# visionworkbench/visionworkbench

Hardware: AMD Instinct MI355X
Metric: disparity Mpix/s, 4096x4096 pair, 7x7 SAD, +-64-px search (higher is better)
Workload: dtype u8

## Files before the change

visionworkbench_amd/csrc/bm_sad_u8.hip:

```cpp
#include <climits>
#include <cstdlib>
#include <type_traits>

#include "vwgpu_internal.h"
#include "u8_tile.h"

#ifdef VWGPU_TILE_STAMPS
__device__ unsigned long long* g_sad_stamps = nullptr;
extern "C" int vwgpu_debug_set_sad_stamps(void* d_buf) {
  unsigned long long* p = static_cast<unsigned long long*>(d_buf);
  return hipMemcpyToSymbol(HIP_SYMBOL(g_sad_stamps), &p, sizeof p) == hipSuccess ? 0 : -3;
}
#define VWGPU_STAMP(k) do { if (g_sad_stamps && tid == 0) g_sad_stamps[(size_t)wg * 16 + (k)] = wall_clock64(); } while (0)
#else
#define VWGPU_STAMP(k) do { } while (0)
#endif

namespace {

using namespace vwgpu_u8;
typedef uint32_t u32;
typedef uint64_t u64;
typedef unsigned short u16x2 __attribute__((ext_vector_type(2)));

__device__ __forceinline__ u32 pk_sub_u16(u32 a, u32 b) {
  return __builtin_bit_cast(u32, (u16x2)(__builtin_bit_cast(u16x2, a) - __builtin_bit_cast(u16x2, b)));
}
__device__ __forceinline__ u32 pk_max_u16(u32 a, u32 b) {
  return __builtin_bit_cast(u32, __builtin_elementwise_max(__builtin_bit_cast(u16x2, a), __builtin_bit_cast(u16x2, b)));
}
__device__ __forceinline__ u32 pk_min_u16(u32 a, u32 b) {
  return __builtin_bit_cast(u32, __builtin_elementwise_min(__builtin_bit_cast(u16x2, a), __builtin_bit_cast(u16x2, b)));
}
__device__ __forceinline__ void umin3_acc(u32& k, u32 a, u32 b) {
  asm volatile("v_min3_u32 %0, %0, %1, %2" : "+v"(k) : "v"(a), "v"(b));
}

template <int W>
__device__ __forceinline__ void key_sub(u32& key, u32 a, u32 b) {
  if (W == 0)
    asm volatile("v_sub_u16_sdwa %0, %1, %2 dst_sel:WORD_1 dst_unused:UNUSED_PRESERVE src0_sel:WORD_0 src1_sel:WORD_0"
                 : "+v"(key) : "v"(a), "v"(b));
  else
    asm volatile("v_sub_u16_sdwa %0, %1, %2 dst_sel:WORD_1 dst_unused:UNUSED_PRESERVE src0_sel:WORD_1 src1_sel:WORD_1"
                 : "+v"(key) : "v"(a), "v"(b));
}

template <int KX, int KY, int TY, int WV = 0>
struct Cfg {
  static constexpr int NW = (KX + 3) / 4;
  static constexpr int EW = NW <= 2 ? 2 : 4;
  static constexpr int WAVES = WV ? WV : (NW <= 2 ? 4 : 2);
  static constexpr int THREADS = WAVES * 64;
  static constexpr int TWB = WAVES * 256;
  static constexpr int NR = TY + KY - 1;
  static constexpr int LBW = TWB / 4 + NW + 1;
  static constexpr u32 LAST_MASK = (KX % 4 == 0) ? 0xffffffffu : ((1u << (8 * (KX % 4))) - 1u);
};

__device__ __forceinline__ void divmod_small(int idx, int d, float inv, int& quo, int& rem) {
  int qq = (int)(((float)idx + 0.5f) * inv);
  int rr = idx - qq * d;
  if (rr < 0) { --qq; rr += d; }
  if (rr >= d) { ++qq; rr -= d; }
  quo = qq; rem = rr;
}

__host__ __device__ constexpr size_t ent_words(int nr, int ne, int ew, int gr, int ty, int pt) {
  const size_t ent = (size_t)nr * ne * ew;
  const size_t merge = gr > 1 ? (size_t)(gr - 1) * (ty / gr) * 4 * pt + (size_t)gr * pt : 0;
  const size_t ob = (size_t)gr * (pt / 64) * 768;
  return ent > merge ? (ent > ob ? ent : ob) : (merge > ob ? merge : ob);
}

template <int KX, int KY, int TY, int GR, int WV = 0, bool EM = true>
__global__ void __launch_bounds__((GR * (Cfg<KX, KY, TY, WV>::THREADS)), (GR > 1 ? 1 : (TY <= 8 && KX <= 8 ? 3 : 2)))
bm_sad_u8_kernel(const float* __restrict__ L, ptrdiff_t ls, int lw, int lh,
                 const float* __restrict__ R, ptrdiff_t rs, int rcw, int rch,
                 int sx, int sy, int ne, int32_t* __restrict__ out, ptrdiff_t os, int ow, int oh,
                 int* __restrict__ flag_set, int* __restrict__ flag_clear,
                 int gxt, int ntiles, int last_round) {
  typedef Cfg<KX, KY, TY, WV> C;
  constexpr bool SPLIT = GR > 1;
  constexpr int NW = C::NW, EW = C::EW, NR = C::NR;
  constexpr int NRP = EM ? (NR | 1) : NR;
  extern __shared__ __attribute__((aligned(16))) u32 lds[];
  u32* ent = lds;
  const int bpitch = ne + NW + 1;
  u32* base = lds + ent_words(NRP, ne, EW, GR, TY, C::THREADS);
  u32* item_ctr = base + (size_t)NR * bpitch;

  constexpr int PT = C::THREADS;
  constexpr int NT = GR * PT;
  const int tid = threadIdx.x;
  const int grp = SPLIT ? __builtin_amdgcn_readfirstlane(tid / PT) : 0;
  const int ltid = SPLIT ? tid % PT : tid;
  const int pair_id = __builtin_amdgcn_readfirstlane(ltid >> 6);
  const int per_xcd = gridDim.x >> 3;
  const int wg = (int)(blockIdx.x & 7) * per_xcd + (int)(blockIdx.x >> 3);
  if (wg >= ntiles) return;
  const int x0 = (wg % gxt) * C::TWB;
  const int y0 = (wg / gxt) * TY;
  const int q = x0 + 4 * ltid;
  u32 bad_acc = 0;
  if (wg == 0 && tid == 0) *flag_clear = 0;
#ifdef VWGPU_TILE_STAMPS
  if (g_sad_stamps && tid == 0) {
    unsigned hw, xcc;
    asm volatile("s_getreg_b32 %0, hwreg(HW_REG_HW_ID)" : "=s"(hw));
    asm volatile("s_getreg_b32 %0, hwreg(HW_REG_XCC_ID)" : "=s"(xcc));
    unsigned long long* rec = g_sad_stamps + (size_t)wg * 16;
    rec[0] = wall_clock64(); rec[1] = clock64(); rec[2] = ((unsigned long long)xcc << 32) | hw;
  }
#endif

  stage_u8_rows<NR>(L, ls, lw, lh, x0, y0, C::LBW, C::LBW, ent, tid, NT, bad_acc);
  stage_u8_rows<NR>(R, rs, rcw, rch, x0, y0, bpitch, bpitch, base, tid, NT, bad_acc);
  __syncthreads();
  u64 win[NR][NW];
#pragma unroll
  for (int r = 0; r < NR; ++r) {
    u32 a[NW + 1];
#pragma unroll
    for (int n = 0; n <= NW; ++n) a[n] = ent[r * C::LBW + ltid + n];
#pragma unroll
    for (int n = 0; n < NW; ++n) win[r][n] = (u64)a[n] | ((u64)a[n + 1] << 32);
  }

  VWGPU_STAMP(3);
  u32 K[TY][4];
  u32 MN[TY][2], MX[TY][2];
#pragma unroll
  for (int y = 0; y < TY; ++y) K[y][0] = K[y][1] = K[y][2] = K[y][3] = 0xffffffffu;
  u32 eq_rows = (1u << TY) - 1u;
  int eq_checks = 0;
  constexpr int NPROBE = 4;
  const u32 zero = 0;

  const bool late = !SPLIT && (int)blockIdx.x >= last_round;
  if (!SPLIT) { if (late) __builtin_amdgcn_s_setprio(2); else __builtin_amdgcn_s_setprio(3); }
  typedef std::true_type T;
  typedef std::false_type F;

  auto sweep = [&](auto max_tag) __attribute__((always_inline)) {
    constexpr bool MAXSWEEP = decltype(max_tag)::value;
    for (int dy = 0; dy < sy; ++dy) {
      __syncthreads();
      if (dy > 0 || (MAXSWEEP && sy > 1)) stage_u8_rows<NR>(R, rs, rcw, rch, x0, y0 + dy, bpitch, bpitch, base, tid, NT, bad_acc);
      for (int t = 0; t < 4; ++t) {
        const int a_last = (sx + 2 - t) >> 2;
        __syncthreads();
        if (!MAXSWEEP && !SPLIT && dy == 0 && late) {
          if (t == 2) __builtin_amdgcn_s_setprio(1);
          else if (t == 3) __builtin_amdgcn_s_setprio(0);
        }
        {
          auto build = [&](int r, int m) __attribute__((always_inline)) {
            const u32* bp = base + (size_t)r * bpitch + m;
            u32 b[NW + 1];
#pragma unroll
            for (int n = 0; n <= NW; ++n) b[n] = bp[n];
            u32 w[EW];
#pragma unroll
            for (int n = 0; n < EW; ++n) w[n] = 0;
#pragma unroll
            for (int n = 0; n < NW; ++n) w[n] = __builtin_amdgcn_alignbyte(b[n + 1], b[n], t);
            w[NW - 1] &= C::LAST_MASK;
            u32* e = ent + (EM ? (size_t)m * NRP + r : (size_t)r * ne + m) * EW;
            if (EW == 2) *reinterpret_cast<uint2*>(e) = make_uint2(w[0], w[1]);
            else *reinterpret_cast<uint4*>(e) = make_uint4(w[0], w[1], w[2 % EW], w[3 % EW]);
          };
#pragma unroll 4
          for (int r = grp; r < NR; r += NT / PT) build(r, ltid);
          const int rem = ne - PT, total = NR * rem;
          const float inv = 1.0f / (float)rem;
          for (int idx = tid; idx < total; idx += NT) {
            int r, m;
            divmod_small(idx, rem, inv, r, m);
            build(r, PT + m);
          }
          if (SPLIT && tid < PT / 64) item_ctr[tid] = 0u;
        }
        __syncthreads();

        auto step = [&](int a, auto masked_tag, auto pair_tag, auto probe_tag) __attribute__((always_inline)) {
          constexpr bool MASKED = decltype(masked_tag)::value;
          constexpr bool PAIR = decltype(pair_tag)::value;
          constexpr bool PROBE = decltype(probe_tag)::value;
          const int jbase = 4 * a + t;
          const int ibase = dy * sx + jbase;
          u32 kinA[4], kinB[4];
          u32 orA[2] = {0u, 0u};
#pragma unroll
          for (int i = 0; i < 4; ++i) {
            kinA[i] = (u32)(ibase - i) & 0xffffu;
            kinB[i] = (u32)(ibase + 4 - i) & 0xffffu;
            if (MASKED) {
              const int d = jbase - i;
              if (d < 0 || d >= sx) orA[i >> 1] |= (i & 1) ? 0xffff0000u : 0x0000ffffu;
            }
          }
          const u32* ep = ent + (size_t)(ltid + a) * (EM ? NRP * EW : EW);
          u64 accA = 0, accB = 0;
          u64 PA[NR], PB[NR];
          constexpr int PF = 4;
          u32 wa[NR][EW], wb[NR][EW];
          auto fetch = [&](int r) __attribute__((always_inline)) {
            const u32* e = ep + (EM ? (size_t)r * EW : (size_t)r * ne * EW);
            constexpr int NX = EM ? NRP * EW : EW;
            if (EW == 2) {
              const uint2 v = *reinterpret_cast<const uint2*>(e);
              wa[r][0] = v.x; wa[r][1] = v.y;
              if (PAIR) { const uint2 u = *reinterpret_cast<const uint2*>(e + NX); wb[r][0] = u.x; wb[r][1] = u.y; }
            } else {
              const uint4 v = *reinterpret_cast<const uint4*>(e);
              wa[r][0] = v.x; wa[r][1] = v.y; wa[r][2 % EW] = v.z; wa[r][3 % EW] = v.w;
              if (PAIR) { const uint4 u = *reinterpret_cast<const uint4*>(e + NX); wb[r][0] = u.x; wb[r][1] = u.y; wb[r][2 % EW] = u.z; wb[r][3 % EW] = u.w; }
            }
          };
#pragma unroll
          for (int r = 0; r < PF && r < NR; ++r) fetch(r);
#pragma unroll
          for (int r = 0; r < NR; ++r) {
            if (r + PF < NR) fetch(r + PF);
#pragma unroll
            for (int n = 0; n < NW; ++n) {
              accA = __builtin_amdgcn_qsad_pk_u16_u8(win[r][n], wa[r][n], accA);
              if (PAIR) accB = __builtin_amdgcn_qsad_pk_u16_u8(win[r][n], wb[r][n], accB);
            }
            PA[r] = accA;
            if (PAIR) PB[r] = accB;
            if (r >= KY - 1) {
              const int y = r - (KY - 1);
              const int ro = (r >= KY) ? r - KY : 0;
              const u32 nA0 = (u32)PA[r], nA1 = (u32)(PA[r] >> 32);
              const u32 oA0 = (r >= KY) ? (u32)PA[ro] : zero;
              const u32 oA1 = (r >= KY) ? (u32)(PA[ro] >> 32) : zero;
              if (MAXSWEEP) {
                const u32 sA0 = pk_sub_u16(nA0, oA0), sA1 = pk_sub_u16(nA1, oA1);
                MN[y][0] = pk_min_u16(MN[y][0], MASKED ? (sA0 | orA[0]) : sA0);
                MN[y][1] = pk_min_u16(MN[y][1], MASKED ? (sA1 | orA[1]) : sA1);
                MX[y][0] = pk_max_u16(MX[y][0], MASKED ? (sA0 & ~orA[0]) : sA0);
                MX[y][1] = pk_max_u16(MX[y][1], MASKED ? (sA1 & ~orA[1]) : sA1);
                if (PAIR) {
                  const u32 nB0 = (u32)PB[r], nB1 = (u32)(PB[r] >> 32);
                  const u32 oB0 = (r >= KY) ? (u32)PB[ro] : zero;
                  const u32 oB1 = (r >= KY) ? (u32)(PB[ro] >> 32) : zero;
                  const u32 sB0 = pk_sub_u16(nB0, oB0), sB1 = pk_sub_u16(nB1, oB1);
                  MN[y][0] = pk_min_u16(MN[y][0], sB0);
                  MN[y][1] = pk_min_u16(MN[y][1], sB1);
                  MX[y][0] = pk_max_u16(MX[y][0], sB0);
                  MX[y][1] = pk_max_u16(MX[y][1], sB1);
                }
              } else {
                key_sub<0>(kinA[0], nA0, oA0); key_sub<1>(kinA[1], nA0, oA0);
                key_sub<0>(kinA[2], nA1, oA1); key_sub<1>(kinA[3], nA1, oA1);
                if (PAIR) {
                  const u32 nB0 = (u32)PB[r], nB1 = (u32)(PB[r] >> 32);
                  const u32 oB0 = (r >= KY) ? (u32)PB[ro] : zero;
                  const u32 oB1 = (r >= KY) ? (u32)(PB[ro] >> 32) : zero;
                  key_sub<0>(kinB[0], nB0, oB0); key_sub<1>(kinB[1], nB0, oB0);
                  key_sub<0>(kinB[2], nB1, oB1); key_sub<1>(kinB[3], nB1, oB1);
                  if (PROBE) {
                    u32 x[4];
#pragma unroll
                    for (int i = 0; i < 4; ++i) {
                      asm volatile("v_xor_b32 %0, %1, %2" : "=v"(x[i]) : "v"(kinA[i]), "v"(kinB[i]));
                      x[i] = (q + i < ow) ? x[i] : 0xffffffffu;
                    }
                    const u32 m01 = x[0] < x[1] ? x[0] : x[1], m23 = x[2] < x[3] ? x[2] : x[3];
                    if ((m01 < m23 ? m01 : m23) >> 16) eq_rows &= ~(1u << y);
                  }
                  umin3_acc(K[y][0], kinA[0], kinB[0]);
                  umin3_acc(K[y][1], kinA[1], kinB[1]);
                  umin3_acc(K[y][2], kinA[2], kinB[2]);
                  umin3_acc(K[y][3], kinA[3], kinB[3]);
                } else {
                  const u32 kA0 = (MASKED && (orA[0] & 0x0000ffffu)) ? 0xffffffffu : kinA[0];
                  const u32 kA1 = (MASKED && (orA[0] & 0xffff0000u)) ? 0xffffffffu : kinA[1];
                  const u32 kA2 = (MASKED && (orA[1] & 0x0000ffffu)) ? 0xffffffffu : kinA[2];
                  const u32 kA3 = (MASKED && (orA[1] & 0xffff0000u)) ? 0xffffffffu : kinA[3];
                  umin3_acc(K[y][0], kA0, kA0);
                  umin3_acc(K[y][1], kA1, kA1);
                  umin3_acc(K[y][2], kA2, kA2);
                  umin3_acc(K[y][3], kA3, kA3);
                }
              }
            }
          }
        };

        int a_lo = (t >= 3) ? 0 : 1;
        int a_hi = (sx - 1 - t >= 0) ? ((sx - 1 - t) >> 2) + 1 : 0;
        if (a_hi > a_last + 1) a_hi = a_last + 1;
        if (a_lo > a_hi) a_lo = a_hi;
        const int n1 = a_lo;
        const int npair = (a_hi - n1) > 0 ? (a_hi - n1) >> 1 : 0;
        int nprobe = 0;
        if (!MAXSWEEP && dy == 0 && t == 0) nprobe = npair < NPROBE - eq_checks ? npair : NPROBE - eq_checks;
        const int a4 = n1 + 2 * npair;
        const int n4 = a_last - a4 + 1 > 0 ? a_last - a4 + 1 : 0;
        const int nitems = n1 + npair + n4;
        int seq = 0;
        auto next_item = [&]() __attribute__((always_inline)) -> int {
          if (MAXSWEEP) return grp == 0 ? seq++ : 0x7fffffff;
          if (!SPLIT) return seq++;
          int lane, v = 0;
          asm volatile("v_mbcnt_lo_u32_b32 %0, -1, 0\n\tv_mbcnt_hi_u32_b32 %0, -1, %0" : "=v"(lane));
          if (lane == 0) v = (int)atomicAdd(&item_ctr[pair_id], 1u);
          return __builtin_amdgcn_readfirstlane(v);
        };
        int i = next_item();
        for (; i < n1; i = next_item()) step(i, T{}, F{}, F{});
        for (; i < n1 + nprobe; i = next_item()) step(n1 + 2 * (i - n1), F{}, T{}, T{});
        for (; i < n1 + npair; i = next_item()) step(n1 + 2 * (i - n1), F{}, T{}, F{});
        for (; i < nitems; i = next_item()) step(a4 + (i - n1 - npair), T{}, F{}, F{});
        eq_checks += nprobe;
        if (!MAXSWEEP && dy == 0) VWGPU_STAMP(4 + t);
      }
    }
  };
  sweep(F{});
  if (!SPLIT) __builtin_amdgcn_s_setprio(3);

  if (bad_acc != 0u) atomicOr(flag_set, 1);
  constexpr int RG = TY / GR;
  static_assert(TY % GR == 0, "rows per group");
  auto row_mine = [&](int y) __attribute__((always_inline)) -> bool { return !SPLIT || (y / RG == grp); };
  if (SPLIT) {
    u32* xk = ent;
    u32* xe = ent + (size_t)(GR - 1) * RG * 4 * PT;
    u32 eq_all = eq_rows;
#pragma unroll
    for (int d = 0; d < GR; ++d) {
      __syncthreads();
      if (grp != d) {
        const int slot = grp < d ? grp : grp - 1;
#pragma unroll
        for (int y = 0; y < RG; ++y)
#pragma unroll
          for (int s2 = 0; s2 < 4; ++s2) xk[((slot * RG + y) * 4 + s2) * PT + ltid] = K[d * RG + y][s2];
      }
      if (d == 0) xe[grp * PT + ltid] = eq_rows;
      __syncthreads();
      if (grp == d) {
#pragma unroll
        for (int slot = 0; slot < GR - 1; ++slot)
#pragma unroll
          for (int y = 0; y < RG; ++y)
#pragma unroll
            for (int s2 = 0; s2 < 4; ++s2) {
              const u32 o = xk[((slot * RG + y) * 4 + s2) * PT + ltid];
              K[d * RG + y][s2] = o < K[d * RG + y][s2] ? o : K[d * RG + y][s2];
            }
      }
      if (d == 0) {
#pragma unroll
        for (int g2 = 0; g2 < GR; ++g2) eq_all &= xe[g2 * PT + ltid];
      }
    }
    eq_rows = eq_all;
  }
  u32 cand = eq_checks < NPROBE ? (1u << TY) - 1u : eq_rows;
#pragma unroll
  for (int y = 0; y < TY; ++y)
    if (y0 + y >= oh || q >= ow || !row_mine(y)) cand &= ~(1u << y);
  const int any = __syncthreads_or(cand != 0u);

  {
    const int wv = ltid >> 6, lane = ltid & 63;
    u32* ob = ent + (size_t)(grp * (PT / 64) + wv) * 768;
    const int xw = x0 + 256 * wv;
    int nd = (ow - xw) * 3;
    nd = nd < 0 ? 0 : (nd > 768 ? 768 : nd);
    const u32 sx_magic = sx > 1 ? (u32)(0xffffffffu / (u32)sx) + 1u : 0u;
    struct __attribute__((packed, aligned(4))) U4 { u32 x, y, z, w; };
#pragma unroll
    for (int y = 0; y < TY; ++y) {
      const int oy = y0 + y;
      if (oy >= oh || !row_mine(y)) continue;
      u32 v[12];
#pragma unroll
      for (int s = 0; s < 4; ++s) {
        const u32 di = K[y][s] & 0xffffu;
        u32 dx, dy;
        if (sy == 1) { dx = di; dy = 0; }
        else { dy = sx == 1 ? di : __umulhi(di, sx_magic); dx = di - dy * (u32)sx; }
        v[3 * s] = dx;
        v[3 * s + 1] = dy;
        v[3 * s + 2] = 0x7fffffffu;
      }
      uint4* ow4 = reinterpret_cast<uint4*>(ob + lane * 12);
      ow4[0] = make_uint4(v[0], v[1], v[2], v[3]);
      ow4[1] = make_uint4(v[4], v[5], v[6], v[7]);
      ow4[2] = make_uint4(v[8], v[9], v[10], v[11]);
      int32_t* orow = out + ((ptrdiff_t)oy * os + xw) * 3;
#pragma unroll
      for (int k = 0; k < 3; ++k) {
        const int idx = k * 256 + lane * 4;
        const uint4 t = *reinterpret_cast<const uint4*>(ob + idx);
        if (idx + 3 < nd) {
          U4 u; u.x = t.x; u.y = t.y; u.z = t.z; u.w = t.w;
          *reinterpret_cast<U4*>(orow + idx) = u;
        } else {
          if (idx < nd) orow[idx] = (int32_t)t.x;
          if (idx + 1 < nd) orow[idx + 1] = (int32_t)t.y;
          if (idx + 2 < nd) orow[idx + 2] = (int32_t)t.z;
        }
      }
    }
  }

#ifdef VWGPU_TILE_STAMPS
  if (g_sad_stamps && tid == 0) { g_sad_stamps[(size_t)wg * 16 + 8] = wall_clock64(); g_sad_stamps[(size_t)wg * 16 + 9] = clock64(); }
#endif
  if (__builtin_expect(!any, 1)) return;
#pragma unroll
  for (int y = 0; y < TY; ++y) {
    MN[y][0] = MN[y][1] = 0xffffffffu;
    MX[y][0] = MX[y][1] = 0u;
  }
  sweep(T{});
  if (grp == 0) {
#pragma unroll
    for (int y = 0; y < TY; ++y) {
      const u32 same0 = MN[y][0] ^ MX[y][0], same1 = MN[y][1] ^ MX[y][1];
      const bool inv[4] = {(same0 & 0xffffu) == 0, (same0 >> 16) == 0, (same1 & 0xffffu) == 0, (same1 >> 16) == 0};
#pragma unroll
      for (int s = 0; s < 4; ++s)
        if (inv[s] && y0 + y < oh && q + s < ow)
          out[((ptrdiff_t)(y0 + y) * os + q + s) * 3 + 2] = 0;
    }
  }
}

typedef void (*KernelFn)(const float*, ptrdiff_t, int, int, const float*, ptrdiff_t, int, int, int, int, int,
                         int32_t*, ptrdiff_t, int, int, int*, int*, int, int, int);
struct Launch {
  int kx, ky, ty;
  int threads, twb, nr, ew, nw;
  int split_groups;
  KernelFn fn;
  KernelFn split_fn;
  KernelFn fn_rm, split_fn_rm;
};

template <bool ON, int KX, int KY, int TY, int GR, int WV, bool EM>
constexpr KernelFn kernel_if() {
  if constexpr (ON) return bm_sad_u8_kernel<KX, KY, TY, GR, WV, EM>;
  else return nullptr;
}

template <int KX, int KY, int TY, bool WITH_SPLIT = false, int WV = 0>
constexpr Launch make_launch() {
  typedef Cfg<KX, KY, TY, WV> C;
  return Launch{KX, KY, TY, C::THREADS, C::TWB, C::NR, C::EW, C::NW, WV ? 4 : 2,
                kernel_if<WV == 0, KX, KY, TY, 1, WV, true>(),
                kernel_if<WITH_SPLIT, KX, KY, TY, (WV ? 4 : 2), WV, true>(),
                kernel_if<WV == 0, KX, KY, TY, 1, WV, false>(),
                kernel_if<WITH_SPLIT, KX, KY, TY, (WV ? 4 : 2), WV, false>()};
}

const Launch kLaunch[] = {
    make_launch<3, 3, 16>(), make_launch<5, 5, 16>(), make_launch<7, 7, 16, true>(), make_launch<7, 7, 8, true>(), make_launch<7, 7, 16, true, 2>(),
    make_launch<7, 5, 16>(), make_launch<9, 9, 12>(), make_launch<11, 11, 8>(),
};

const Launch* find_launch(int kx, int ky) {
  for (const Launch& l : kLaunch)
    if (l.kx == kx && l.ky == ky) return &l;
  return nullptr;
}

const Launch* pick_launch(int kx, int ky, int ow, int oh, int num_cu, int groups, bool* split) {
  const Launch* best = nullptr;
  double best_cost = 0.0;
  *split = false;
  if (groups == 3) {
    bool has = false;
    for (const Launch& l : kLaunch) has |= l.kx == kx && l.ky == ky && l.split_fn && !l.fn;
    if (!has) groups = 0;
  }
  for (const Launch& l : kLaunch) {
    if (l.kx != kx || l.ky != ky) continue;
    const long long wgs = (long long)((ow + l.twb - 1) / l.twb) * ((oh + l.ty - 1) / l.ty);
    const double n = (double)((wgs + num_cu - 1) / num_cu);
    const int resident = (l.ty <= 8 && l.kx <= 8) ? 3 : 2;
    const bool narrow = l.twb * 2 <= 4 * 256 && l.split_fn && !l.fn;
    const double wfrac = narrow ? 0.5 : 1.0;
    for (int sp = 0; sp < 2; ++sp) {
      if (sp && !l.split_fn) continue;
      if (!sp && !l.fn) continue;
      if (groups == 3 && !narrow) continue;
      if (groups && groups != 3 && (narrow || (l.split_fn && (groups == 2) != (sp == 1)))) continue;
      const double steps = (sp ? l.nr * 0.55 * n : (n < 2.0 ? l.nr * 0.74 : l.nr * 0.5 * n)) * wfrac;
      const double rounds = sp ? n : (double)(((long long)n + resident - 1) / resident);
      const double cost = steps + (narrow ? 5.7 : 4.5) * rounds;
      if (!best || cost < best_cost) { best = &l; best_cost = cost; *split = sp != 0; }
    }
  }
  return best;
}

constexpr size_t kMaxLds = 80 * 1024;

int entries_per_row(const Launch& l, int sx) { return l.twb / 4 + ((sx + 2) >> 2) + 1; }

size_t lds_bytes(const Launch& l, int sx, int groups, bool em) {
  const int ne = entries_per_row(l, sx);
  const size_t ent = ent_words(em ? (l.nr | 1) : l.nr, ne, l.ew, groups, l.ty, l.threads);
  const size_t left = (size_t)l.nr * (l.twb / 4 + l.nw + 1);
  const size_t base = (size_t)l.nr * (ne + l.nw + 1);
  return ((ent > left ? ent : left) + base) * sizeof(u32);
}

}

bool vwgpu_bm_sad_u8_supported(int cost_type, int kx, int ky, int sx, int sy) {
  if (cost_type != VWGPU_ABSOLUTE_DIFFERENCE) return false;
  const Launch* l = find_launch(kx, ky);
  if (!l) return false;
  if ((long long)sx * sy > 65535) return false;
  return lds_bytes(*l, sx, l->split_fn ? l->split_groups : 1, false) <= kMaxLds;
}

int vwgpu_launch_bm_sad_u8(vwgpu_ctx* ctx,
                           const float* left, int lw, int lh, ptrdiff_t ls,
                           const float* right, int rw, int rh, ptrdiff_t rs,
                           int kx, int ky, int sx, int sy, int32_t* out, ptrdiff_t os,
                           int** d_fallback_flag) {
  (void)rw; (void)rh;
  const int ow = lw - kx + 1, oh = lh - ky + 1;
  bool split = false;
  const Launch* l = pick_launch(kx, ky, ow, oh, ctx->num_cu, ctx->sad_groups, &split);
  if (!l) return vwgpu_fail(ctx, VWGPU_ERR_NOIMPL, "no packed-u8 kernel for %dx%d", kx, ky);
  const int rcw = lw + sx - 1, rch = lh + sy - 1;
  const int gx = (ow + l->twb - 1) / l->twb, gy = (oh + l->ty - 1) / l->ty;
  const int ne = entries_per_row(*l, sx);

  int *flag_set = nullptr, *flag_clear = nullptr;
  int rc = vwgpu_next_flags(ctx, 0, &flag_set, &flag_clear, nullptr);
  if (rc) return rc;
  *d_fallback_flag = flag_set;
  const int groups = split ? l->split_groups : 1;
  const size_t ctr_bytes = split ? 64 : 0;
  const bool em = ctx->sad_layout == 0 && lds_bytes(*l, sx, groups, true) + ctr_bytes <= kMaxLds;
  const size_t shmem = lds_bytes(*l, sx, groups, em) + ctr_bytes;
  ctx->sad_last_launch = l->ty | (l->twb / 256) << 8 | groups << 12 | (em ? 1 : 0) << 16;
  const KernelFn main_fn = em ? (split ? l->split_fn : l->fn) : (split ? l->split_fn_rm : l->fn_rm);
  const unsigned grid1 = (unsigned)((gx * gy + 7) / 8 * 8);
  const int slots = ctx->num_cu * ((l->ty <= 8 && l->kx <= 8) ? 3 : 2);
  const int last_round = (!split && (int)grid1 >= 2 * slots) ? (int)grid1 - slots : INT_MAX;
  if (shmem > 64 * 1024)
    VWGPU_HIP(ctx, hipFuncSetAttribute(reinterpret_cast<const void*>(main_fn),
                                       hipFuncAttributeMaxDynamicSharedMemorySize, (int)shmem));
  {
    vwgpu_prof_scope ps(ctx, "bm_sad_u8");
    hipLaunchKernelGGL(main_fn, dim3(grid1), dim3(split ? l->split_groups * l->threads : l->threads), shmem, ctx->stream,
                       left, ls, lw, lh, right, rs, rcw, rch, sx, sy, ne, out, os, ow, oh,
                       flag_set, flag_clear, gx, gx * gy, last_round);
  }
  VWGPU_HIP(ctx, hipGetLastError());
  return VWGPU_OK;
}
```

Measured before the change: 51390.

## Pair masked edge steps and exit equality probes early when no rows remain

Edge (masked) disparity steps are now processed in pairs alongside the clean ones, with per-lane masks OR'd into the keys for the second half, so the schedule has about half as many single masked steps. The probe loop checks with a wave-wide ballot whether any lane still has candidate equal rows and stops probing once none do. eq_rows is also initialised from the valid output range so out-of-bounds lanes do not keep probing alive. This adds OR instructions to masked paths and a rewritten item index mapping that carries risk in the SPLIT work-stealing path.

```diff
diff --git a/visionworkbench_amd/csrc/bm_sad_u8.hip b/visionworkbench_amd/csrc/bm_sad_u8.hip
--- a/visionworkbench_amd/csrc/bm_sad_u8.hip
+++ b/visionworkbench_amd/csrc/bm_sad_u8.hip
@@ -44,6 +44,10 @@
   else
     asm volatile("v_sub_u16_sdwa %0, %1, %2 dst_sel:WORD_1 dst_unused:UNUSED_PRESERVE src0_sel:WORD_1 src1_sel:WORD_1"
                  : "+v"(key) : "v"(a), "v"(b));
+}
+
+__device__ __forceinline__ void key_or(u32& key, u32 m) {
+  asm volatile("v_or_b32 %0, %1, %0" : "+v"(key) : "s"(m));
 }
 
 template <int KX, int KY, int TY, int WV = 0>
@@ -132,7 +136,7 @@
   u32 MN[TY][2], MX[TY][2];
 #pragma unroll
   for (int y = 0; y < TY; ++y) K[y][0] = K[y][1] = K[y][2] = K[y][3] = 0xffffffffu;
-  u32 eq_rows = (1u << TY) - 1u;
+  u32 eq_rows = q < ow ? (oh - y0 >= TY ? (1u << TY) - 1u : (1u << (oh - y0)) - 1u) : 0u;
   int eq_checks = 0;
   constexpr int NPROBE = 4;
   const u32 zero = 0;
@@ -190,14 +194,16 @@
           const int jbase = 4 * a + t;
           const int ibase = dy * sx + jbase;
           u32 kinA[4], kinB[4];
-          u32 orA[2] = {0u, 0u};
+          u32 orA[2] = {0u, 0u}, orB[2] = {0u, 0u};
+          u32 mkA[4] = {0u, 0u, 0u, 0u}, mkB[4] = {0u, 0u, 0u, 0u};
 #pragma unroll
           for (int i = 0; i < 4; ++i) {
             kinA[i] = (u32)(ibase - i) & 0xffffu;
             kinB[i] = (u32)(ibase + 4 - i) & 0xffffu;
             if (MASKED) {
               const int d = jbase - i;
-              if (d < 0 || d >= sx) orA[i >> 1] |= (i & 1) ? 0xffff0000u : 0x0000ffffu;
+              if (d < 0 || d >= sx) { orA[i >> 1] |= (i & 1) ? 0xffff0000u : 0x0000ffffu; mkA[i] = 0xffffffffu; }
+              if (PAIR && (d + 4 < 0 || d + 4 >= sx)) { orB[i >> 1] |= (i & 1) ? 0xffff0000u : 0x0000ffffu; mkB[i] = 0xffffffffu; }
             }
           }
           const u32* ep = ent + (size_t)(ltid + a) * (EM ? NRP * EW : EW);
@@ -247,10 +253,10 @@
                   const u32 oB0 = (r >= KY) ? (u32)PB[ro] : zero;
                   const u32 oB1 = (r >= KY) ? (u32)(PB[ro] >> 32) : zero;
                   const u32 sB0 = pk_sub_u16(nB0, oB0), sB1 = pk_sub_u16(nB1, oB1);
-                  MN[y][0] = pk_min_u16(MN[y][0], sB0);
-                  MN[y][1] = pk_min_u16(MN[y][1], sB1);
-                  MX[y][0] = pk_max_u16(MX[y][0], sB0);
-                  MX[y][1] = pk_max_u16(MX[y][1], sB1);
+                  MN[y][0] = pk_min_u16(MN[y][0], MASKED ? (sB0 | orB[0]) : sB0);
+                  MN[y][1] = pk_min_u16(MN[y][1], MASKED ? (sB1 | orB[1]) : sB1);
+                  MX[y][0] = pk_max_u16(MX[y][0], MASKED ? (sB0 & ~orB[0]) : sB0);
+                  MX[y][1] = pk_max_u16(MX[y][1], MASKED ? (sB1 & ~orB[1]) : sB1);
                 }
               } else {
                 key_sub<0>(kinA[0], nA0, oA0); key_sub<1>(kinA[1], nA0, oA0);
@@ -264,43 +270,50 @@
                   if (PROBE) {
                     u32 x[4];
 #pragma unroll
-                    for (int i = 0; i < 4; ++i) {
-                      asm volatile("v_xor_b32 %0, %1, %2" : "=v"(x[i]) : "v"(kinA[i]), "v"(kinB[i]));
-                      x[i] = (q + i < ow) ? x[i] : 0xffffffffu;
-                    }
-                    const u32 m01 = x[0] < x[1] ? x[0] : x[1], m23 = x[2] < x[3] ? x[2] : x[3];
-                    if ((m01 < m23 ? m01 : m23) >> 16) eq_rows &= ~(1u << y);
+                    for (int i = 0; i < 4; ++i) asm volatile("v_xor_b32 %0, %1, %2" : "=v"(x[i]) : "v"(kinA[i]), "v"(kinB[i]));
+                    u32 m = x[0];
+                    asm("v_min3_u32 %0, %0, %1, %2" : "+v"(m) : "v"(x[1]), "v"(x[2]));
+                    m = m < x[3] ? m : x[3];
+                    if (m >> 16) eq_rows &= ~(1u << y);
+                  }
+                  if (MASKED) {
+#pragma unroll
+                    for (int i = 0; i < 4; ++i) { key_or(kinA[i], mkA[i]); key_or(kinB[i], mkB[i]); }
                   }
                   umin3_acc(K[y][0], kinA[0], kinB[0]);
                   umin3_acc(K[y][1], kinA[1], kinB[1]);
                   umin3_acc(K[y][2], kinA[2], kinB[2]);
                   umin3_acc(K[y][3], kinA[3], kinB[3]);
                 } else {
-                  const u32 kA0 = (MASKED && (orA[0] & 0x0000ffffu)) ? 0xffffffffu : kinA[0];
-                  const u32 kA1 = (MASKED && (orA[0] & 0xffff0000u)) ? 0xffffffffu : kinA[1];
-                  const u32 kA2 = (MASKED && (orA[1] & 0x0000ffffu)) ? 0xffffffffu : kinA[2];
-                  const u32 kA3 = (MASKED && (orA[1] & 0xffff0000u)) ? 0xffffffffu : kinA[3];
-                  umin3_acc(K[y][0], kA0, kA0);
-                  umin3_acc(K[y][1], kA1, kA1);
-                  umin3_acc(K[y][2], kA2, kA2);
-                  umin3_acc(K[y][3], kA3, kA3);
+                  if (MASKED) {
+#pragma unroll
+                    for (int i = 0; i < 4; ++i) key_or(kinA[i], mkA[i]);
+                  }
+                  umin3_acc(K[y][0], kinA[0], kinA[0]);
+                  umin3_acc(K[y][1], kinA[1], kinA[1]);
+                  umin3_acc(K[y][2], kinA[2], kinA[2]);
+                  umin3_acc(K[y][3], kinA[3], kinA[3]);
                 }
               }
             }
           }
         };
 
-        int a_lo = (t >= 3) ? 0 : 1;
-        int a_hi = (sx - 1 - t >= 0) ? ((sx - 1 - t) >> 2) + 1 : 0;
-        if (a_hi > a_last + 1) a_hi = a_last + 1;
-        if (a_lo > a_hi) a_lo = a_hi;
-        const int n1 = a_lo;
-        const int npair = (a_hi - n1) > 0 ? (a_hi - n1) >> 1 : 0;
+        const int nstep = a_last + 1;
+        const int a_lo = (t >= 3) ? 0 : 1;
+        const int a_hi = (sx - 1 - t >= 0) ? ((sx - 1 - t) >> 2) + 1 : 0;
+        const int nsingle = nstep & 1;
+        const int a_single = a_lo ? 0 : nstep - 1;
+        const int p0 = nsingle & a_lo;
+        const int npair = nstep >> 1;
+        const int kc0 = a_lo & ~p0;
+        int kc1 = a_hi - p0 > 0 ? (a_hi - p0) >> 1 : 0;
+        if (kc1 < kc0) kc1 = kc0;
+        const int nclean = kc1 - kc0;
+        const int pc0 = p0 + 2 * kc0;
         int nprobe = 0;
-        if (!MAXSWEEP && dy == 0 && t == 0) nprobe = npair < NPROBE - eq_checks ? npair : NPROBE - eq_checks;
-        const int a4 = n1 + 2 * npair;
-        const int n4 = a_last - a4 + 1 > 0 ? a_last - a4 + 1 : 0;
-        const int nitems = n1 + npair + n4;
+        if (!MAXSWEEP && dy == 0 && t == 0) nprobe = nclean < NPROBE - eq_checks ? nclean : NPROBE - eq_checks;
+        const int nitems = npair + nsingle;
         int seq = 0;
         auto next_item = [&]() __attribute__((always_inline)) -> int {
           if (MAXSWEEP) return grp == 0 ? seq++ : 0x7fffffff;
@@ -310,12 +323,21 @@
           if (lane == 0) v = (int)atomicAdd(&item_ctr[pair_id], 1u);
           return __builtin_amdgcn_readfirstlane(v);
         };
+        const int nprobe0 = nprobe;
         int i = next_item();
-        for (; i < n1; i = next_item()) step(i, T{}, F{}, F{});
-        for (; i < n1 + nprobe; i = next_item()) step(n1 + 2 * (i - n1), F{}, T{}, T{});
-        for (; i < n1 + npair; i = next_item()) step(n1 + 2 * (i - n1), F{}, T{}, F{});
-        for (; i < nitems; i = next_item()) step(a4 + (i - n1 - npair), T{}, F{}, F{});
-        eq_checks += nprobe;
+        for (; i < nprobe; i = next_item()) {
+          step(pc0 + 2 * i, F{}, T{}, T{});
+          if (!SPLIT && __builtin_amdgcn_ballot_w64(eq_rows != 0u) == 0ull) {
+            eq_checks = NPROBE - nprobe;
+            nprobe = 0;
+          }
+        }
+        for (; i < nclean; i = next_item()) step(pc0 + 2 * i, F{}, T{}, F{});
+        for (; i < npair; i = next_item()) {
+          step(p0 + 2 * (i - nclean < kc0 ? 0 : i), T{}, T{}, F{});
+        }
+        for (; i < nitems; i = next_item()) step(a_single, T{}, F{}, F{});
+        eq_checks += nprobe0;
         if (!MAXSWEEP && dy == 0) VWGPU_STAMP(4 + t);
       }
     }
```

Result: no change. 51690 (median of 6 runs) (+0.6%).
